# ranrandy/gaussian-splatting-mpm

Measured on AMD Instinct MI355X. Metric: MPM substeps/sec (and particles·steps/sec) + rendered fps, lego 128³ grid, higher is better.
Workload: dtype f32; 1 GPU; lego.json frame: 100 substeps + postprocess + render 800x800 SH3; particles_per_gpu=100000, particles_total=100000, n_grid=128, material=jelly, render_overlap=True, render_first=False, render_thread=True, render_async=False, parallelism=single

## Files before the change

gaussian-splatting-mpm_amd/csrc/fused.h:

```cpp

#ifndef GSMPM_FT2
#define GSMPM_FT2 7
#endif
constexpr int kFT0 = 8, kFT1 = 8, kFT2 = GSMPM_FT2;
constexpr int kFW0 = kFT0 + 4, kFW1 = kFT1 + 4, kFW2 = kFT2 + 4;
constexpr int kFWin = kFW0 * kFW1 * kFW2;
constexpr int kFTN = kFT0 * kFT1 * kFT2;

__device__ __forceinline__ int slot_loc(int w0, int w1, int w2) { return (w0 * kFW1 + w1) * kFW2 + w2; }

struct SlabWin {
  int W;
  int a[2];
  int on[2];
  float4* part[2];
  int y0[2], ny[2];
  int z0[2], nz[2];
  int* oob;
  int pass;
};

__device__ __forceinline__ int slab_window_of(const SlabWin& sw, int i) {
  if (sw.on[0] && i >= sw.a[0] && i < sw.a[0] + sw.W) return 0;
  if (sw.on[1] && i >= sw.a[1] && i < sw.a[1] + sw.W) return 1;
// ... 219 lines not shown
  int* touched;
  int* nchunk;
  int4* chunk;
  int* cbox;
  int* tbox;
  unsigned char* perm;
  int2* rcov;
  const int* tpos;
  int* rbox;
};

__device__ __forceinline__ int balanced_lane(const int* __restrict__ rcnt, int cnt, int r, int rank) {
  const int Lr = (cnt - r + 15) >> 4;
  if (rank < Lr) return rank * 16 + r;
  int o = rank - Lr;
  for (int q = 0; q < r; ++q) o += max(0, rcnt[q] - ((cnt - q + 15) >> 4));
  int acc = 0;
  for (int q = 0; q < 16; ++q) {
    const int Lq = (cnt - q + 15) >> 4, d = max(0, Lq - rcnt[q]);
    if (o < acc + d) return (rcnt[q] + (o - acc)) * 16 + q;
    acc += d;
  }
  return rank * 16 + r;
}

constexpr int kFullBox = 0 | (0 << 4) | (0 << 8) | ((kFW0 - 1) << 12) | ((kFW1 - 1) << 16) | ((kFW2 - 1) << 20);
__device__ __forceinline__ void box_unpack(int b, int (&lo)[3], int (&hi)[3]) {
#pragma unroll
  for (int d = 0; d < 3; ++d) {
    lo[d] = (b >> (4 * d)) & 15;
    hi[d] = (b >> (12 + 4 * d)) & 15;
  }
}

__device__ __forceinline__ void add_lower_tiles(const Touch& tc, const FTiles& tl, int tx, int ty, int tz, int lo) {
  const int e = threadIdx.x;
  if (e < 27) {
    const int a = e / 9 - 1, b = (e / 3) % 3 - 1, c = e % 3 - 1;
    const bool need = (a < 0 || b < 0 || c < 0) && (a >= 0 || (lo & 1)) && (b >= 0 || (lo & 2)) && (c >= 0 || (lo & 4));
    const int x = tx + a, y = ty + b, z = tz + c;
    if (need && (unsigned)x < (unsigned)tl.td0 && (unsigned)y < (unsigned)tl.td1 && (unsigned)z < (unsigned)tl.td2) {
      const int t = (x * tl.td1 + y) * tl.td2 + z;
      if (atomicCAS(&tc.tflag[t], 0, 1) == 0) {
        const int pos = atomicAdd(&tc.nchunk[1], 1);
        tc.touched[pos] = t;
        if (tc.rcov) tc.rcov[(size_t)pos * kRecStride + 27] = make_int2(1, 0);
      }
    }
  }
}

__device__ __forceinline__ void base_of(const float (&x)[3], float inv_dx, int (&b)[3]) {
#pragma unroll
  for (int d = 0; d < 3; ++d) b[d] = (int)(x[d] * inv_dx - 0.5f);
}

__device__ __forceinline__ void mark_escape_tiles(int* __restrict__ tflag, int* __restrict__ touched,
                                               int* __restrict__ ntouch, int2* __restrict__ rcov, const FTiles& tl,
                                               int ng, int b0, int b1, int b2) {
  const int lo0 = max(b0, 0), lo1 = max(b1, 0), lo2 = max(b2, 0);
  const int hi0 = min(b0 + 2, ng - 1), hi1 = min(b1 + 2, ng - 1), hi2 = min(b2 + 2, ng - 1);
  if (lo0 > hi0 || lo1 > hi1 || lo2 > hi2) return;
  for (int a = lo0 / kFT0; a <= hi0 / kFT0; ++a)
    for (int c = lo1 / kFT1; c <= hi1 / kFT1; ++c)
      for (int e = lo2 / kFT2; e <= hi2 / kFT2; ++e) {
        const int t = (a * tl.td1 + c) * tl.td2 + e;
// ... 66 lines not shown
}

__global__ __launch_bounds__(1024) void k_fold_tail(int* __restrict__ flags, float4* __restrict__ g0,
                                                    float4* __restrict__ g1, float4* __restrict__ g2, int ng) {
  __shared__ int s_f[12];
  if (threadIdx.x < 12) s_f[threadIdx.x] = flags[threadIdx.x];
  __syncthreads();
  const size_t nn = (size_t)ng * ng * ng;
  bool dirty[3] = {false, false, false};
  for (int r = 0; r < 12; ++r) dirty[r % 3] = dirty[r % 3] || s_f[r] != 0;
  float4* gb[3] = {g0, g1, g2};
  for (int b = 0; b < 3; ++b)
    if (dirty[b])
      for (size_t q = threadIdx.x; q < nn; q += 1024) gb[b][q] = make_float4(0.f, 0.f, 0.f, 0.f);
  __syncthreads();
  if (threadIdx.x < 12 && s_f[threadIdx.x]) flags[threadIdx.x] = 0;
}

__device__ __forceinline__ void load_cover27(const ChunkIn& ck, const int* __restrict__ tbox, const FTiles& tl, int ti,
                                             int tj, int tk, int* s_cov, int* s_bx) {
  const int e = threadIdx.x;
  if (e < 27) {
    const int x = ti + e / 9 - 1, y = tj + (e / 3) % 3 - 1, z = tk + e % 3 - 1;
    int c0 = 0, nc = 0, bx = 0;
    if ((unsigned)x < (unsigned)tl.td0 && (unsigned)y < (unsigned)tl.td1 && (unsigned)z < (unsigned)tl.td2) {
      const int t = (x * tl.td1 + y) * tl.td2 + z;
      const int cnt = ck.count[t];
      c0 = ck.cbase[t];
      bx = tbox[t];
      nc = (cnt + kChunk - 1) / kChunk;
    }
    s_cov[2 * e] = c0;
    s_cov[2 * e + 1] = nc;
    s_bx[e] = bx;
  }
}

struct NodeReads {
  int off[8];
  int extra;
  int live;
};
__device__ __forceinline__ void node_cover(int l0, int l1, int l2, int e, int& ci, int& loc) {
  const int sec0 = l0 < 3 ? -1 : (l0 == kFT0 - 1 ? 1 : 0);
  const int sec1 = l1 < 3 ? -1 : (l1 == kFT1 - 1 ? 1 : 0);
  const int sec2 = l2 < 3 ? -1 : (l2 == kFT2 - 1 ? 1 : 0);
  const int a = (e >> 2) ? sec0 : 0, b = ((e >> 1) & 1) ? sec1 : 0, c = (e & 1) ? sec2 : 0;
  ci = (a + 1) * 9 + (b + 1) * 3 + (c + 1);
  loc = slot_loc(l0 - a * kFT0 + 1, l1 - b * kFT1 + 1, l2 - c * kFT2 + 1);
}
__device__ __forceinline__ void node_reads(int max_chunks, const int* s_cov, const int* s_bx, int l0,
                                           int l1, int l2, NodeReads& r) {
  const int sec0 = l0 < 3 ? -1 : (l0 == kFT0 - 1 ? 1 : 0);
  const int sec1 = l1 < 3 ? -1 : (l1 == kFT1 - 1 ? 1 : 0);
  const int sec2 = l2 < 3 ? -1 : (l2 == kFT2 - 1 ? 1 : 0);
  r.extra = 0;
  r.live = 0;
  int nc[8], bx[8], c0[8], ci[8];
#pragma unroll
  for (int e = 0; e < 8; ++e) {
    const int a = (e >> 2) ? sec0 : 0, b = ((e >> 1) & 1) ? sec1 : 0, c = (e & 1) ? sec2 : 0;
    ci[e] = (a + 1) * 9 + (b + 1) * 3 + (c + 1);
    nc[e] = s_cov[2 * ci[e] + 1];
    bx[e] = s_bx[ci[e]];
    c0[e] = s_cov[2 * ci[e]];
  }
#pragma unroll
  for (int e = 0; e < 8; ++e) {
    const int ax = e >> 2, ay = (e >> 1) & 1, az = e & 1;
    const int a = ax ? sec0 : 0, b = ay ? sec1 : 0, c = az ? sec2 : 0;
    const int w0 = l0 - a * kFT0 + 1, w1 = l1 - b * kFT1 + 1, w2 = l2 - c * kFT2 + 1;
    const int q = bx[e];
    const bool on = ((!ax) | (sec0 != 0)) & ((!ay) | (sec1 != 0)) & ((!az) | (sec2 != 0)) & (nc[e] > 0) &
                    (w0 >= (q & 15)) & (w1 >= ((q >> 4) & 15)) & (w2 >= ((q >> 8) & 15)) &
                    (w0 <= ((q >> 12) & 15)) & (w1 <= ((q >> 16) & 15)) & (w2 <= ((q >> 20) & 15));
    const int loc = slot_loc(w0, w1, w2);
    r.off[e] = on ? c0[e] * kFWin + loc : max_chunks * kFWin;
    r.extra |= (on & (nc[e] > 1)) ? (1 << e) : 0;
    r.live |= on ? (1 << e) : 0;
  }
}
__device__ __forceinline__ void add4(float4& a, const float4& b) {
  a.x += b.x;
  a.y += b.y;
  a.z += b.z;
  a.w += b.w;
}
__device__ __forceinline__ void glds4(const int* src, int* lds_base) {
  __builtin_amdgcn_global_load_lds((const __attribute__((address_space(1))) void*)src,
                                   (__attribute__((address_space(3))) void*)lds_base, 4, 0, 0);
}
__device__ __forceinline__ float4 ld_slot(const float4* __restrict__ slots, int off) {
  return *(const float4*)((const char*)slots + (unsigned)off * 16u);
}
#ifndef GSMPM_STREAM_BATCH
#define GSMPM_STREAM_BATCH 8
#endif
constexpr int kStreamBatch = GSMPM_STREAM_BATCH;
__device__ __forceinline__ void node_extra(const float4* __restrict__ slots, const int* s_cov, int l0,
                                           int l1, int l2, int extra2, int zero, float4& acc) {
  int runs = extra2;
#pragma unroll
  for (int e = 0; e < 8; ++e) {
    int ci, loc;
    node_cover(l0, l1, l2, e, ci, loc);
    runs |= (((extra2 >> e) & 1) & (s_cov[2 * ci + 1] > 2)) << (8 + e);
  }
  const int sec0 = l0 < 3 ? -1 : (l0 == kFT0 - 1 ? 1 : 0);
// ... 50 lines not shown
    P = wt / kGridParts;
    part = wt - P * kGridParts;
  } else {
    const int x = b & 7, m = (b >> 3) + it * (S >> 3);
    const int u = m / kGridParts, k = u / kGridGroup;
    part = m - u * kGridParts;
    P = (k * 8 + x) * kGridGroup + (u - k * kGridGroup);
  }
}
template <bool SLAB, bool EXT = false, class GS = GridStep>
__global__ __launch_bounds__(kGridT) __attribute__((amdgpu_waves_per_eu(7, 8))) void k_grid_f(GridDims g, FTiles tl, ChunkIn ck, const int* __restrict__ tbox,
                                                    const float4* __restrict__ slots, float4* __restrict__ gacc,
                                                    float4* __restrict__ gvel, const BcTable* __restrict__ bct,
                                                    GS gs, const int* __restrict__ esc_in,
                                                    int* __restrict__ esc_clear, int* __restrict__ zc,
                                                    int* __restrict__ zf, SlabWin sw) {
  sim_prio();
  stamp(3, 0);
  const int pass = SLAB ? sw.pass : 0;
  int P0, part0;
  grid_work(blockIdx.x, 0, gridDim.x, P0, part0);
  const int i0 = min(P0, tl.ntiles - 1);
  const int* esc_p = esc_in;
  const int* cnt_p = ck.nchunk;
  const int* tch_p = ck.touched;
  asm volatile("" : "+s"(esc_p), "+s"(cnt_p), "+s"(tch_p));
  const bool pre = ck.rcov != nullptr;
  const int le = threadIdx.x;
  __shared__ int s_rec[2][64];
  __shared__ int s_box[2][64];
  __shared__ int s_tn[2];
  if (pre && threadIdx.x < 64) {
    glds4(reinterpret_cast<const int*>(ck.rcov) + (size_t)i0 * 2 * kRecStride + le, &s_rec[0][0]);
    glds4(ck.rbox + (size_t)i0 * kRecStride + (le & 31), &s_box[0][0]);
  }
  typedef const int __attribute__((address_space(1)))* gint_p;
  const int esc0 = __builtin_amdgcn_readfirstlane(*(gint_p)esc_p);
  const int cnt0 = __builtin_amdgcn_readfirstlane(((gint_p)cnt_p)[1]);
  const int T0 = __builtin_amdgcn_readfirstlane(((gint_p)tch_p)[i0]);
  const int ng = g.ng;
  const bool esc = esc0 != 0;
  const int ntouch = cnt0;
  int b = 0;
  for (int it = 0;; ++it, b ^= 1) {
    int P, part;
    grid_work(blockIdx.x, it, gridDim.x, P, part);
    if (P >= ntouch) break;
    asm volatile("s_waitcnt vmcnt(0)" ::: "memory");
    __syncthreads();
    int pn, partn;
    grid_work(blockIdx.x, it + 1, gridDim.x, pn, partn);
    if (pre && pn < ntouch && threadIdx.x < 64) {
      glds4(reinterpret_cast<const int*>(ck.rcov) + (size_t)pn * 2 * kRecStride + le, &s_rec[b ^ 1][0]);
      glds4(ck.rbox + (size_t)pn * kRecStride + (le & 31), &s_box[b ^ 1][0]);
      if (le == 0) glds4(ck.touched + pn, &s_tn[b ^ 1]);
    }
    int* s_cov = s_rec[b];
    int* s_bx = s_box[b];
    const int q = threadIdx.x + part * kGridT;
    const int l0 = q / (kFT1 * kFT2), l1 = (q / kFT2) % kFT1, l2 = q % kFT2;
    const int T = it == 0 ? T0 : pre ? s_tn[b] : ck.touched[P];
    if ((unsigned)T >= (unsigned)tl.ntiles) continue;
    int ti, tj, tk;
    ftile_decode(tl, T, ti, tj, tk);
    if (SLAB && pass != 0 && slab_tile_in_window(sw, ti) != (pass == 1)) continue;
    if (it == 0) stamp(3, 2);
    const bool tables = !pre || s_cov[54] != 0;
    if (tables) {
      load_cover27(ck, tbox, tl, ti, tj, tk, s_cov, s_bx);
      __syncthreads();
    }
    if (it == 0) stamp(3, 3);
#ifdef GSMPM_STAMPS
    if (it == 0 && threadIdx.x == 0) {
      int ncmax = 0;
      for (int e = 0; e < 27; ++e) ncmax = max(ncmax, s_cov[2 * e + 1]);
      stamp_val(3, 5, (unsigned long long)T);
      stamp_val(3, 6, (unsigned long long)(s_cov[2 * 13 + 1] | (ncmax << 16)));
      stamp_val(3, 7, (unsigned long long)part);
    }
#endif
    const int i = ti * kFT0 + l0, j = tj * kFT1 + l1, k = tk * kFT2 + l2;
    if ((unsigned)i < (unsigned)ng && (unsigned)j < (unsigned)ng && (unsigned)k < (unsigned)ng) {
      const size_t idx = ((size_t)i * ng + j) * ng + k;
      float4 a = make_float4(0.f, 0.f, 0.f, 0.f);
      NodeReads r;
      node_reads(tl.max_chunks, s_cov, s_bx, l0, l1, l2, r);
// ... 57 lines not shown
```

gaussian-splatting-mpm_amd/csrc/fused_body.inc:

```
#ifndef GSMPM_FUSED_BODY_INCLUDER
#error "fused_body.inc is the body of k_fused / k_fused_mixed: it is included inside those two kernels in fused.h only"
#endif
  constexpr bool G2P = (MODE & 1) != 0, P2G = (MODE & 2) != 0;
  constexpr bool FOLD = G2P && (MODE & 4) != 0;
  __shared__ int s_fc0[27], s_fnc[27], s_fbx[27];
  constexpr int kEscMax = kFWin / 27;
  __shared__ int s_nesc;
  __shared__ int s_eb[3][kEscMax];
  GridStep fgs{};
  bool fesc = false;
  if constexpr (FOLD) {
    fgs.dt = dt;
    fgs.dgx = dt * rare->grav[0];
    fgs.dgy = dt * rare->grav[1];
    fgs.dgz = dt * rare->grav[2];
    fgs.mask = mask_prev;
    fgs.keep = 0;
    fesc = __builtin_amdgcn_readfirstlane(*rare->esc_prev) != 0;
  }
  __shared__ unsigned long long s_acc[4 * kFWin];
  __shared__ float s_max[4];
  __shared__ int s_mxy[4], s_mz[4];
  __shared__ int s_cnt[27], s_base[27];
  __shared__ int s_rcnt[16];
  float4* s_win = reinterpret_cast<float4*>(s_acc);
  const int ng = g.ng;
  constexpr int SK = (MODE & 3) == 3 ? 0 : 1;
  sim_prio();
  stamp(SK, 0);
  const int w0 = min((int)blockIdx.x, tl.max_chunks - 1);
  const bool perm0 = use_box && tc.perm;
  const int* nch_p = ck.nchunk;
  const int4* chk_p = ck.chunk;
  const int* cbx_p = tc.cbox;
  const unsigned char* prm_p = perm0 ? tc.perm : reinterpret_cast<const unsigned char*>(tc.cbox);
  asm volatile("" : "+s"(nch_p), "+s"(chk_p), "+s"(cbx_p), "+s"(prm_p));
  typedef const int __attribute__((address_space(1)))* gint_p;
  typedef const unsigned char __attribute__((address_space(1)))* guc_p;
  const gint_p c4 = (gint_p)chk_p + 4 * (size_t)w0;
  const int r0 = c4[0], r1 = c4[1], r2 = c4[2], r3 = c4[3];
  const int bx0 = ((gint_p)cbx_p)[w0];
  const int qv0 = ((guc_p)prm_p)[perm0 ? (size_t)w0 * 256 + threadIdx.x : 0];
  const int nch = *(gint_p)nch_p;
  int4 cr_n = make_int4(r0, r1, r2, r3);
  int box_n = use_box ? bx0 : kFullBox;
  int q_n = perm0 ? qv0 : (int)threadIdx.x;
  for (int w = blockIdx.x; w < nch; w += gridDim.x) {
    const int4 cr = cr_n;
    const int cbox = box_n, q_lane = q_n;
    if (w + (int)gridDim.x < nch) {
      const int wn = w + gridDim.x;
      cr_n = ck.chunk[wn];
      box_n = use_box ? tc.cbox[wn] : kFullBox;
      q_n = (use_box && tc.perm) ? (int)tc.perm[(size_t)wn * 256 + threadIdx.x] : (int)threadIdx.x;
    }
    const int t = cr.x, first = cr.y, cnt = cr.z;
    const int k = threadIdx.x;
    const bool outside = t == tl.ntiles;
    int tx = 0, ty = 0, tz = 0;
    if (!outside) ftile_decode(tl, t, tx, ty, tz);
    const int o0 = tx * kFT0 - 1, o1 = ty * kFT1 - 1, o2 = tz * kFT2 - 1;
    int tpos_e = -1;
    const int* __restrict__ tposp = rare->tpos;
    if (tposp && !outside && k < 27) {
      const int x0 = tx - (k / 9 - 1), y0 = ty - ((k / 3) % 3 - 1), z0 = tz - (k % 3 - 1);
      if ((unsigned)x0 < (unsigned)tl.td0 && (unsigned)y0 < (unsigned)tl.td1 && (unsigned)z0 < (unsigned)tl.td2)
        tpos_e = tposp[(x0 * tl.td1 + y0) * tl.td2 + z0];
    }
    int p = -1;
    float x[3] = {0.f, 0.f, 0.f}, v[3] = {0.f, 0.f, 0.f}, C[3][3], F[3][3], m = 0.f;
    const int q = k >= cnt ? k : q_lane;
    if (k < cnt) {
      p = first + q;
#pragma unroll
      for (int d = 0; d < 3; ++d) x[d] = ps.ld(PX + d, p);
      if (G2P || MAT != 0) {
#pragma unroll
        for (int i = 0; i < 9; ++i) F[i / 3][i % 3] = ps.ld(PF + i, p);
      }
      if (P2G) m = ps.ld(PMASS, p);
      if (!G2P) {
#pragma unroll
        for (int d = 0; d < 3; ++d) v[d] = ps.ld(PV + d, p);
#pragma unroll
        for (int i = 0; i < 9; ++i) C[i / 3][i % 3] = ps.ld(PC + i, p);
      }
    }
// ... 336 lines not shown
        for (int o = 32; o > 0; o >>= 1) {
          bound = fmaxf(bound, __shfl_xor(bound, o));
          mxy |= __shfl_xor(mxy, o);
          mz |= __shfl_xor(mz, o);
        }
      }
      if ((k & 63) == 0) {
        s_max[k >> 6] = bound;
        s_mxy[k >> 6] = mxy;
        s_mz[k >> 6] = mz;
      }
      __syncthreads();
      const int res = win ? (((b[0] - o0) * kFW1 + (b[1] - o1)) * kFW2 + (b[2] - o2)) & 15 : (q & 15);
      const int rrank = (tc.perm && k < cnt) ? atomicAdd(&s_rcnt[res], 1) : 0;
      const float bmax = fmaxf(fmaxf(s_max[0], s_max[1]), fmaxf(s_max[2], s_max[3]));
      const int Mxy = s_mxy[0] | s_mxy[1] | s_mxy[2] | s_mxy[3], Mz = s_mz[0] | s_mz[1] | s_mz[2] | s_mz[3];
      const int Mx = Mxy & 0xffff, My = (unsigned)Mxy >> 16;
      const int lo_all = (Mx & 1) | ((My & 1) << 1) | ((Mz & 1) << 2);
      if (lo_all & ~cr.w) {
        Touch tr = tc;
        tr.tflag = rare->tflag;
        tr.touched = rare->touched;
        tr.nchunk = rare->nchunk;
        tr.rcov = rare->rcov;
        add_lower_tiles(tr, tl, tx, ty, tz, (lo_all | cr.w) & 7);
        if (k == 0) rare->chunk[w].w = lo_all | cr.w;
      }
      int box = kFullBox;
      if (Mx && My && Mz)
        box = (__builtin_ctz(Mx)) | (__builtin_ctz(My) << 4) | (__builtin_ctz(Mz) << 8) | ((31 - __builtin_clz(Mx)) << 12) |
              ((31 - __builtin_clz(My)) << 16) | ((31 - __builtin_clz(Mz)) << 20);
      else
        box = 0;
      if (k == 0) {
        tc.cbox[w] = box;
        rare->tbox[t] = (cr.w & 8) ? kFullBox : box;
      }
      if (tpos_e >= 0) rare->rbox[(size_t)tpos_e * kRecStride + k] = (cr.w & 8) ? kFullBox : box;
      if (cr.w & 8) box = kFullBox;
      int ebits;
      frexpf(bmax, &ebits);
      const int S = bmax > 0.f ? 50 - ebits : 0;
      if (k < cnt) {
        if (win) {
          int bb[3];
          float fx[3], ww[3][3], dw[3][3];
          bspline(x, g.inv_dx, bb, fx, ww, dw);
          p2g_scatter<MAT, kFW1, kFW2, kFWin>(s_acc + ((b[0] - o0) * kFW1 + (b[1] - o1)) * kFW2 + (b[2] - o2), fx, ww,
                                              dw, v, C, m, nvt, g, dt, ldexp(1.0, S));
        } else {
          p2g_global<MAT>(x, v, C, m, nvt, g, dt, rare->gacc);
          *rare->esc = 1;
        }
      }
      {
        const unsigned long long eb = __ballot(k < cnt && !win);
        if (eb) {
          if ((k & 63) == 0) atomicAdd(rare->esc_count, (unsigned)__popcll(eb));
          if (k < cnt && !win)
            mark_escape_tiles(rare->tflag, rare->touched, rare->nchunk + 1, rare->rcov, tl, ng, b[0], b[1], b[2]);
        }
      }
      __syncthreads();
      if (w == (int)blockIdx.x) stamp(SK, 4);
      if (tc.perm && k < cnt) tc.perm[(size_t)w * 256 + balanced_lane(s_rcnt, cnt, res, rrank)] = (unsigned char)q;
      int lo[3], hi[3];
      box_unpack(box, lo, hi);
      const int n1 = hi[1] - lo[1] + 1, n2 = hi[2] - lo[2] + 1, n12 = n1 * n2;
      const int nvol = (hi[0] - lo[0] + 1) * n12;
      const float r12 = 1.0f / (float)n12, r2 = 1.0f / (float)n2;
      const int cid = (cr.w & 16) ? (int)((unsigned)cr.w >> 5) : w;
      float4* dst = slots + (size_t)cid * kFWin;
// ... 31 lines not shown
```

gaussian-splatting-mpm_amd/csrc/mpm.hip:

```cpp
#include <hip/hip_runtime.h>
#include <dlfcn.h>


#include <algorithm>
#include <climits>
#include <cmath>
#include <cstring>
#include <map>
#include <numeric>
#include <type_traits>
#include <vector>

#include "common.h"
#include "constitutive.h"
#include <hip/hip_ext.h>

#include "mpm_common.h"
#include "svd3.h"

namespace gsmpm {

#ifndef GSMPM_REBIN_SF
#define GSMPM_REBIN_SF 20
#endif
// ... 856 lines not shown
    __syncthreads();
    if (w == (int)blockIdx.x) stamp(1, 4);
    if (p >= 0) {
      bo.ptile[p] = nt;
      bo.pslot[p] = code >= 0 ? s_base[code] + lslot : reserve(bo, nt, 1);
    }
    __syncthreads();
  }
  stamp(1, 1);
}

__global__ __launch_bounds__(256) void k_bin_all(Particles ps, GridDims g, Tiles tl, BinOut bo) {
  const int p = blockIdx.x * blockDim.x + threadIdx.x;
  if (p < ps.n) {
    float x[3];
#pragma unroll
    for (int d = 0; d < 3; ++d) x[d] = ps.ld(PX + d, p);
    int tc[3];
    const int t = tile_of(x, g, tl, tc);
    bo.ptile[p] = t;
    bo.pslot[p] = reserve(bo, t, 1);
  }
}

struct ChunkOut {
  int* cstart;
  int* cbase;
  int4* chunk;
  int* nchunk;
  const int* tflag;
  int* touched;
  int2* rcov = nullptr;
  int* tpos = nullptr;
  int td1 = 0, td2 = 0;
};

constexpr int kRecStride = 32;
__device__ __forceinline__ void write_cover_record(const ChunkOut& co, int ntiles, int E, int t, int rk,
                                                   const int* s_off, const int* s_aux, int total) {
  const int td12 = co.td1 * co.td2, td0 = ntiles / td12;
  const int tz = t % co.td2, ty = (t / co.td2) % co.td1, tx = t / td12;
  for (int e = 0; e < 27; ++e) {
    const int x = tx + e / 9 - 1, y = ty + (e / 3) % 3 - 1, z = tz + e % 3 - 1;
    int2 r = make_int2(0, 0);
    if ((unsigned)x < (unsigned)td0 && (unsigned)y < (unsigned)co.td1 && (unsigned)z < (unsigned)co.td2) {
      const int u = (x * co.td1 + y) * co.td2 + z;
      const int cnt = (u + 1 < E ? s_off[u + 1] : total) - s_off[u];
      r = make_int2(s_aux[u] & 0xffff, (cnt + kChunk - 1) / kChunk);
    }
    co.rcov[(size_t)rk * kRecStride + e] = r;
  }
  co.rcov[(size_t)rk * kRecStride + 27] = make_int2(0, 0);
}

__device__ __forceinline__ int wave_incl_scan(int v) {
  const int lane = threadIdx.x & 63;
#pragma unroll
  for (int o = 1; o < 64; o <<= 1) {
    const int y = __shfl_up(v, o);
    if (lane >= o) v += y;
  }
  return v;
}

__device__ __forceinline__ void block_scan3(const int (&v)[3], int (&o)[3], int (&tot)[3]) {
  __shared__ int s_ws[3][4];
  const int lane = threadIdx.x & 63, wave = threadIdx.x >> 6;
#pragma unroll
  for (int r = 0; r < 3; ++r) {
    const int inc = wave_incl_scan(v[r]);
    if (lane == 63) s_ws[r][wave] = inc;
    o[r] = inc - v[r];
  }
  __syncthreads();
#pragma unroll
  for (int r = 0; r < 3; ++r) {
    tot[r] = 0;
#pragma unroll
    for (int w = 0; w < 4; ++w) {
      if (w < wave) o[r] += s_ws[r][w];
      tot[r] += s_ws[r][w];
    }
  }
// ... 594 lines not shown
  int* ptile = nullptr;
  int* pslot = nullptr;
  int cur_box = 0;
  BcTable host_bc{};
  BcTable* dev_bc = nullptr;
  int n_bc = 0;
  int n_ext = 0;
  int n_mov = 0;
  float* times_dev = nullptr;
  int times_cap = 0;
  int n_rot = 0;
  RotRec host_rot[kMaxBC] = {};
  RotRec* rot_dev = nullptr;
  float* poses_dev = nullptr;
  int poses_rot = 0, poses_n = 0;
  bool has_particles = false;
  bool has_R = false;
  hipStream_t cap = nullptr;
  int resort_interval = 100;
  long since_sort = 0;
  float* planes_tmp = nullptr;
  int* orig_tmp = nullptr;
  uint32_t* sort_keys = nullptr;
  int* sort_idx = nullptr;
  unsigned* sort_tmp = nullptr;
  bool fused = true;
  FTiles ftl{};
  bool fold = false;
  bool rebin_auto = false;
  int rebin_m = 0;
  bool lane_balance = true;
  bool fuse_permute = true;
  bool cover_records = true;
  int fused_wgs = 1024;
  bool chunk_order = true;
  int ncu = 256;
  int fbpar = 0;
  int fep = 0;
  int rebin_interval = 10;
  std::map<std::vector<uint32_t>, hipGraphExec_t> graphs;
  std::map<std::vector<uint32_t>, hipGraphExec_t> graphs_alt;
  std::map<std::vector<uint32_t>, int> graph_turn;
  int graph_copies = 1;
  std::map<std::vector<uint32_t>, int> graph_box_parity;
  struct FState {
    int bpar, ep;
    float* planes;
    float* planes_alt;
    int* orig;
    int* orig_alt;
    float* cold;
    float* cold_alt;
    int* gid;
    int* gid_alt;
    long since, migrations;
  };
  std::map<std::vector<uint32_t>, FState> graph_fstate;
  bool slab = false;
  int s_lo = 0, s_hi = 0, s_margin = 2, s_interval = 10, s_rank = 0, s_world = 1;
  int s_has[2] = {0, 0};
  SlabWin sw{};
  float4* s_recv[2] = {nullptr, nullptr};
  int* d_n = nullptr;
  int* s_drift = nullptr;
  bool s_synced = false;
  bool s_rect_set = false;
// ... 92 lines not shown
static ChunkOut chunk_out(const BinLists& b) {
  return ChunkOut{b.cstart, b.cbase, b.chunk, b.nchunk, b.tflag, b.touched};
}

static ChunkIn chunk_in(gsmpm_mpm* h, int c) { return chunk_in(h->ph.b[c], h->ph.b[c].chunk); }
static ChunkOut chunk_out(gsmpm_mpm* h, int c) { return chunk_out(h->ph.b[c]); }
static BinOut bin_out(gsmpm_mpm* h, int c) {
  return BinOut{h->ph.b[c].count, h->ptile, h->pslot, h->ph.b[c].tflag, h->tl.td, h->tl.ntiles};
}

static bool use_fused(const gsmpm_mpm* h) { return h->fused; }
static const BinLists& bin_lists(const gsmpm_mpm* h, int c) { return use_fused(h) ? h->fu.b[c] : h->ph.b[c]; }

static int kernel_code(const gsmpm_mpm* h) { return h->mixed ? kMatMixed : h->mat_kernel; }
static MatIds<kMatMixed> mat_ids_of(gsmpm_mpm* h) {
  return MatIds<kMatMixed>{h->mat_ids, h->orig, (h->prm.flags & GSMPM_FLAG_JELLY_FCR) ? 4 : 0};
}

static int4* fused_records(gsmpm_mpm* h, int c) {
  return h->chunk_order ? h->fu.pchunk[c] : h->fu.b[c].chunk;
}
static ChunkIn chunk_in_f(gsmpm_mpm* h, int c) {
  ChunkIn ci = chunk_in(h->fu.b[c], fused_records(h, c));
  if (h->cover_records) {
    ci.rcov = h->fu.rcov[c];
    ci.rbox = h->fu.rbox[c];
  }
  return ci;
}
static ChunkOut chunk_out_f(gsmpm_mpm* h, int c) {
  ChunkOut co = chunk_out(h->fu.b[c]);
  co.rcov = h->fu.rcov[c];
  co.tpos = h->fu.tpos[c];
  co.td1 = h->ftl.td1;
  co.td2 = h->ftl.td2;
  return co;
}
static Touch touch_f(gsmpm_mpm* h, int c) {
  const BinLists& b = h->fu.b[c];
  return Touch{b.tflag, b.touched, b.nchunk, b.chunk, h->fu.cbox[c], h->fu.tbox[c],
               h->lane_balance ? h->fu.perm[c] : nullptr, h->fu.rcov[c],
               h->cover_records ? h->fu.tpos[c] : nullptr, h->fu.rbox[c]};
}
static BinOutF bin_out_f(gsmpm_mpm* h, int c) {
  return BinOutF{h->fu.b[c].count, h->ptile, h->pslot, h->fu.b[c].tflag, h->ftl};
}
static Tiles ftiles_flat(const gsmpm_mpm* h) { return Tiles{h->ftl.td0, h->ftl.ntiles, h->ftl.max_chunks}; }

static int p2g_grid(gsmpm_mpm* h) { return std::min(h->tl.max_chunks, 1024); }
static int g2p_grid(gsmpm_mpm* h) { return std::min(h->tl.max_chunks, 1024); }
static int grid_grid(gsmpm_mpm* h) { return std::min(h->tl.ntiles, 1024); }

template <typename F, typename... Args>
static void launch(const hipEvent_t* ev, F kernel, dim3 grid, dim3 block, hipStream_t st, Args... args) {
  if (ev)
    hipExtLaunchKernelGGL(kernel, grid, block, 0, st, ev[0], ev[1], 0, args...);
  else
    hipLaunchKernelGGL(kernel, grid, block, 0, st, args...);
}

template <int MAT>
static void launch_p2g(gsmpm_mpm* h, int c, uint32_t mask, float dt, hipStream_t st, const hipEvent_t* ev) {
  if constexpr (MAT == kMatMixed)
    launch(ev, k_p2g_mixed, dim3(p2g_grid(h)), dim3(kChunk), st, particles_of(h), h->g, h->tl, chunk_in(h, c),
           (const BcTable*)h->dev_bc, mask, dt, h->mc, h->ph.slots, h->gacc, h->nonfin_dev, mat_ids_of(h));
  else
// ... 341 lines not shown
    r.gacc_old = fold_gacc(h, ph - 2);
    r.esc_clr = fold_flag(h, ph - 3);
  }
  for (int d = 0; d < 3; ++d) r.grav[d] = (float)h->prm.gravity[d];
  r.esc_count = reinterpret_cast<unsigned*>(h->fu.esc + 3 + kFoldPhases);
  r.esc_nodes = h->fo.esc_nodes;
  r.vmax = h->slab ? nullptr : h->fu.vmax_dev;
  return r;
}
static int sync_rare(gsmpm_mpm* h, hipStream_t st) {
  bool dirty = false;
  for (int i = 0; i < 2 * kRareSlots; ++i) {
    if (i % kRareSlots >= 2 && !h->fold) continue;
    const FusedRare r = rare_of(h, i / kRareSlots, i % kRareSlots);
    if (std::memcmp(&r, &h->frare_host[i], sizeof(r)) != 0) {
      h->frare_host[i] = r;
      dirty = true;
    }
  }
  if (!dirty) return GSMPM_OK;
  GSMPM_REQUIRE(!h->capturing, "k_fused's rare arguments changed inside a capture");
  GSMPM_HIP(hipMemcpyAsync(h->fu.rare_dev, h->frare_host, sizeof(h->frare_host), hipMemcpyHostToDevice, st));
  return GSMPM_OK;
}
struct FusedLaunch {
  int c, bin, use_box, slot;
  uint32_t mask, mask_prev;
  float dt;
  float4* slots;
};
template <int MAT, int MODE>
static void launch_fused_t(gsmpm_mpm* h, const FusedLaunch& f, hipStream_t st, const hipEvent_t* ev) {
  const int xlo = h->slab ? h->s_lo - h->s_margin : INT_MIN, xhi = h->slab ? h->s_hi + h->s_margin : INT_MAX;
  if constexpr (MAT == kMatMixed)
    launch(ev, k_fused_mixed<MODE>, dim3(fused_grid(h)), dim3(256), st, particles_of(h), h->g, h->ftl,
           chunk_in_f(h, f.c), touch_f(h, f.c), f.bin, f.use_box, (const float4*)h->gvel, f.mask, f.dt, h->mc, f.slots,
           xlo, xhi, (const FusedRare*)(h->fu.rare_dev + f.c * kRareSlots + f.slot), f.mask_prev, mat_ids_of(h));
  else
    launch(ev, k_fused<MAT, MODE>, dim3(fused_grid(h)), dim3(256), st, particles_of(h), h->g, h->ftl,
           chunk_in_f(h, f.c), touch_f(h, f.c), f.bin, f.use_box, (const float4*)h->gvel, f.mask, f.dt, h->mc, f.slots,
           xlo, xhi, (const FusedRare*)(h->fu.rare_dev + f.c * kRareSlots + f.slot), f.mask_prev);
}
template <int MODE>
static void launch_fused_m(gsmpm_mpm* h, const FusedLaunch& f, hipStream_t st, const hipEvent_t* ev) {
  switch (kernel_code(h)) {
    case 0: launch_fused_t<0, MODE>(h, f, st, ev); break;
    case 1: launch_fused_t<1, MODE>(h, f, st, ev); break;
    case 2: launch_fused_t<2, MODE>(h, f, st, ev); break;
    case 3: launch_fused_t<3, MODE>(h, f, st, ev); break;
    case 5: launch_fused_t<5, MODE>(h, f, st, ev); break;
    case kMatMixed:
      if constexpr ((MODE & 4) == 0) launch_fused_t<kMatMixed, MODE>(h, f, st, ev);
      break;
    default: launch_fused_t<4, MODE>(h, f, st, ev); break;
  }
}
static int launch_fused(gsmpm_mpm* h, int mode, const FusedLaunch& f, hipStream_t st, const hipEvent_t* ev) {
  if (!h->capturing) {
    const int rc = sync_rare(h, st);
    if (rc) return rc;
  }
  switch (mode) {
    case 1: launch_fused_t<0, 1>(h, f, st, ev); break;
    case 5: launch_fused_t<0, 5>(h, f, st, ev); break;
    case 2: launch_fused_m<2>(h, f, st, ev); break;
    case 7: launch_fused_m<7>(h, f, st, ev); break;
    default: launch_fused_m<3>(h, f, st, ev); break;
  }
  GSMPM_LAUNCH_CHECK();
  return GSMPM_OK;
}
static int launch_fused(gsmpm_mpm* h, int mode, int c, bool bin, bool use_box, uint32_t mask, float dt, int ep,
                        hipStream_t st, const hipEvent_t* ev) {
// ... 485 lines not shown
  h->g.ng = prm->n_grid;
  h->g.dx = (float)(prm->grid_extent / prm->n_grid);
  h->g.inv_dx = (float)(prm->n_grid / prm->grid_extent);
  const double sin_phi = std::sin(prm->friction_angle_deg / 180.0 * 3.141592653589793);
  h->mc.alpha = (float)(std::sqrt(2.0 / 3.0) * 2.0 * sin_phi / (3.0 - sin_phi));
  h->mc.hardening = (float)prm->hardening;
  h->mc.xi = (float)prm->xi;
  h->mc.pvisc = (float)prm->plastic_viscosity;
  h->mat_kernel = prm->material;
  if (prm->material == 0 && (prm->flags & GSMPM_FLAG_JELLY_FCR)) h->mat_kernel = 4;
  h->rebin_interval = h->mat_kernel == 0 ? kRebinStressFree : kRebinStress;
  const size_t nn = (size_t)h->g.ng * h->g.ng * h->g.ng;
  auto fail = [&](hipError_t e, const char* what) {
    set_error(std::string("gsmpm_mpm_create: ") + what + ": " + hipGetErrorString(e));
    gsmpm_mpm_destroy(h);
    return GSMPM_EHIP;
  };
  hipError_t e;
#define GSMPM_TRY(call, what) \
  if ((e = (call)) != hipSuccess) return fail(e, what)
  GSMPM_TRY(alloc(h, &h->planes, (size_t)NPLANES * h->np, kMemCommon, kFillZero), "planes");
  GSMPM_TRY(alloc(h, &h->cold, (size_t)NCOLD * h->np, kMemCommon, kFillZero), "planes");
  GSMPM_TRY(alloc(h, &h->orig, (size_t)h->np, kMemCommon), "orig");
  GSMPM_TRY(alloc(h, &h->gacc, nn, kMemCommon, kFillZero), "grid acc");
  GSMPM_TRY(alloc(h, &h->gvel, nn, kMemCommon, kFillZero), "grid vel");
  h->tl.td = (h->g.ng + kTile - 1) / kTile;
  h->tl.ntiles = h->tl.td * h->tl.td * h->tl.td;
  h->tl.max_chunks = h->n / kChunk + std::min(h->tl.ntiles + 1, h->n) + 1;
  h->fused = !(prm->flags & (GSMPM_FLAG_PHASED | GSMPM_FLAG_KEEP_GRID));
  if (const char* lb = std::getenv("GSMPM_LANE_BALANCE")) h->lane_balance = lb[0] != '0';
  if (const char* gc = std::getenv("GSMPM_GRAPH_COPIES")) h->graph_copies = std::max(1, std::atoi(gc));
  if (const char* fp = std::getenv("GSMPM_FUSE_PERMUTE")) h->fuse_permute = fp[0] != '0';
  if (const char* cr = std::getenv("GSMPM_COVER_RECORDS")) h->cover_records = cr[0] != '0';
  {
    int dev = 0, ncu = 0, per_cu = 0;
    if (hipGetDevice(&dev) == hipSuccess &&
        hipDeviceGetAttribute(&ncu, hipDeviceAttributeMultiprocessorCount, dev) == hipSuccess &&
        hipOccupancyMaxActiveBlocksPerMultiprocessor(&per_cu, k_fused<0, 3>, 256, 0) == hipSuccess && ncu > 0 &&
        per_cu > 0) {
      h->ncu = ncu;
      const int resident = ncu * per_cu;
      const int rounds = (int)std::min<long long>(6, std::max<long long>(1, (long long)h->n / ((long long)resident * kChunk)));
      h->fused_wgs = resident * rounds;
      h->chunk_order = rounds == 1;
    }
    if (const char* fw = std::getenv("GSMPM_FUSED_WGS")) h->fused_wgs = std::max(1, std::atoi(fw));
    if (const char* co = std::getenv("GSMPM_CHUNK_ORDER")) h->chunk_order = co[0] != '0';
  }
  h->ftl.td0 = (h->g.ng + kFT0 - 1) / kFT0;
  h->ftl.td1 = (h->g.ng + kFT1 - 1) / kFT1;
  h->ftl.td2 = (h->g.ng + kFT2 - 1) / kFT2;
  h->ftl.ntiles = h->ftl.td0 * h->ftl.td1 * h->ftl.td2;
  h->ftl.max_chunks = h->n / kChunk + std::min(h->ftl.ntiles + 1, h->n) + 1;
  if (h->fused && sizeof(float4) * (size_t)(h->ftl.max_chunks + 1) * kFWin > 0xffffffffull) h->fused = false;
  if (const char* fo = std::getenv("GSMPM_FOLD")) h->fold = h->fused && fo[0] != '0';
  if (const char* ra = std::getenv("GSMPM_REBIN_AUTO")) h->rebin_auto = h->fused && ra[0] != '0';
  if (!h->fused) {
    GSMPM_TRY(alloc(h, &h->ph.slots, (size_t)(h->tl.max_chunks + 1) * kWin, kMemPhased, kFillZero,
                    (size_t)h->tl.max_chunks * kWin),
              "chunk slots");
    for (BinLists& b : h->ph.b)
      GSMPM_TRY(alloc_bin_lists(h, b, h->tl.ntiles, h->tl.max_chunks, kMemPhased), "bin lists");
  } else {
    FusedBufs& f = h->fu;
    const size_t nt = (size_t)h->ftl.ntiles, mc = (size_t)h->ftl.max_chunks;
    GSMPM_TRY(alloc(h, &f.slots, (mc + 1) * kFWin, kMemFused, kFillZero, mc * kFWin), "fused slots");
    for (int c = 0; c < 2; ++c) {
      GSMPM_TRY(alloc_bin_lists(h, f.b[c], h->ftl.ntiles, h->ftl.max_chunks, kMemFused), "bin lists");
      GSMPM_TRY(alloc(h, &f.cbox[c], mc, kMemFused), "boxes");
      GSMPM_TRY(alloc(h, &f.pchunk[c], mc, kMemFused, kFillZero), "ordered chunks");
      GSMPM_TRY(alloc(h, &f.tbox[c], nt, kMemFused), "boxes");
      GSMPM_TRY(alloc(h, &f.rcov[c], kRecStride * nt, kMemFused, kFillZero), "cover records");
      GSMPM_TRY(alloc(h, &f.rbox[c], kRecStride * nt, kMemFused, kFillZero), "cover boxes");
      GSMPM_TRY(alloc(h, &f.tpos[c], nt, kMemFused, kFillOnes), "touched positions");
      GSMPM_TRY(alloc(h, &f.perm[c], mc * 256, kMemFused, kFillZero), "lane balance");
    }
    GSMPM_TRY(alloc(h, &f.planes_alt, (size_t)NPLANES * h->np, kMemFused, kFillZero), "planes");
    GSMPM_TRY(alloc(h, &f.orig_alt, (size_t)h->np, kMemFused), "orig");
    GSMPM_TRY(alloc(h, &f.esc, 4 + kFoldPhases, kMemFused, kFillZero), "escape flags");
    GSMPM_TRY(alloc(h, &f.vmax_dev, 1, kMemFused, kFillZero), "vmax");
    GSMPM_TRY(alloc_host(h, &f.vmax_host, 1), "pinned vmax");
    *f.vmax_host = 0.f;
    GSMPM_TRY(alloc(h, &f.rare_dev, 2 * kRareSlots, kMemFused, kFillZero), "rare args");
    if (h->fold) {
      GSMPM_TRY(alloc(h, &h->fo.slots2, (mc + 1) * kFWin, kMemFold, kFillZero, mc * kFWin), "fused slots");
      for (float4*& g : h->fo.gacc) GSMPM_TRY(alloc(h, &g, nn, kMemFold, kFillZero), "grid acc");
      GSMPM_TRY(alloc(h, &h->fo.esc_nodes, 27 * (size_t)h->np, kMemFold), "escape nodes");
      for (int*& t : h->fo.tbox2) GSMPM_TRY(alloc(h, &t, nt, kMemFold, kFillZero), "boxes");
    }
  }
  const int scan_tiles = std::max(h->tl.ntiles, h->ftl.ntiles) + 1;
  GSMPM_TRY(alloc(h, &h->scan_part, (size_t)div_up(scan_tiles, 1024), kMemCommon), "scan partials");
  GSMPM_TRY(alloc(h, &h->ptile, (size_t)h->np, kMemCommon), "ptile");
  GSMPM_TRY(alloc(h, &h->pslot, (size_t)h->np, kMemCommon), "pslot");
  GSMPM_TRY(alloc(h, &h->dev_bc, 1, kMemCommon), "bc table");
  GSMPM_TRY(hipStreamCreateWithFlags(&h->cap, hipStreamNonBlocking), "hipStreamCreate");
  GSMPM_TRY(alloc_host(h, &h->nonfin_host, 16, hipHostMallocMapped), "pinned non-finite word");
  *(volatile int*)h->nonfin_host = 0;
  GSMPM_TRY(hipHostGetDevicePointer((void**)&h->nonfin_dev, h->nonfin_host, 0), "hipHostGetDevicePointer");
  h->host_bc = BcTable{};
  GSMPM_TRY(hipMemcpy(h->dev_bc, &h->host_bc, sizeof(BcTable), hipMemcpyHostToDevice), "hipMemcpy bc");
  GSMPM_TRY(hipDeviceSynchronize(), "init");
#undef GSMPM_TRY
  *out = h;
  return GSMPM_OK;
}
// ... 840 lines not shown
```

Baseline: 3.528 billion particle-substeps/s.

## Use per-axis bitmask boxes and hull-merged multi-chunk boxes to skip empty node reads

Cover boxes are now stored as per-axis occupancy bitmasks (x|y<<16, z), so the node-read test becomes shifts and ANDs instead of six range comparisons. Tiles covered by several chunks no longer fall back to a full box. Each chunk ORs its mask into the record atomically, and the running box becomes the hull of the chunk boxes, so more empty window nodes are skipped when gathering. This doubles the cover-box record stride, adds atomics and zeroing writes, and loads 64 ints per record instead of 32. It is enabled by default except in fold mode.

Measured after the change: 3.684 billion particle-substeps/s, median of 6. 4.4% higher.

```diff
diff --git a/gaussian-splatting-mpm_amd/csrc/fused.h b/gaussian-splatting-mpm_amd/csrc/fused.h
--- a/gaussian-splatting-mpm_amd/csrc/fused.h
+++ b/gaussian-splatting-mpm_amd/csrc/fused.h
@@ -275,6 +275,21 @@
     hi[d] = (b >> (12 + 4 * d)) & 15;
   }
 }
+__device__ __forceinline__ int box_hull(int a, int b) {
+  int r = 0;
+#pragma unroll
+  for (int d = 0; d < 3; ++d) {
+    r |= min((a >> (4 * d)) & 15, (b >> (4 * d)) & 15) << (4 * d);
+    r |= max((a >> (12 + 4 * d)) & 15, (b >> (12 + 4 * d)) & 15) << (12 + 4 * d);
+  }
+  return r;
+}
+__device__ __forceinline__ int2 box_masks(int b) {
+  int lo[3], hi[3];
+  box_unpack(b, lo, hi);
+  const int mx = (2 << hi[0]) - (1 << lo[0]), my = (2 << hi[1]) - (1 << lo[1]), mz = (2 << hi[2]) - (1 << lo[2]);
+  return make_int2(mx | (my << 16), mz);
+}
 
 __device__ __forceinline__ void add_lower_tiles(const Touch& tc, const FTiles& tl, int tx, int ty, int tz, int lo) {
   const int e = threadIdx.x;
@@ -407,7 +422,9 @@
     }
     s_cov[2 * e] = c0;
     s_cov[2 * e + 1] = nc;
-    s_bx[e] = bx;
+    const int2 bm = box_masks(bx);
+    s_bx[e] = bm.x;
+    s_bx[32 + e] = bm.y;
   }
 }
 
@@ -431,13 +448,14 @@
   const int sec2 = l2 < 3 ? -1 : (l2 == kFT2 - 1 ? 1 : 0);
   r.extra = 0;
   r.live = 0;
-  int nc[8], bx[8], c0[8], ci[8];
+  int nc[8], bxy[8], bz[8], c0[8], ci[8];
 #pragma unroll
   for (int e = 0; e < 8; ++e) {
     const int a = (e >> 2) ? sec0 : 0, b = ((e >> 1) & 1) ? sec1 : 0, c = (e & 1) ? sec2 : 0;
     ci[e] = (a + 1) * 9 + (b + 1) * 3 + (c + 1);
     nc[e] = s_cov[2 * ci[e] + 1];
-    bx[e] = s_bx[ci[e]];
+    bxy[e] = s_bx[ci[e]];
+    bz[e] = s_bx[32 + ci[e]];
     c0[e] = s_cov[2 * ci[e]];
   }
 #pragma unroll
@@ -445,10 +463,8 @@
     const int ax = e >> 2, ay = (e >> 1) & 1, az = e & 1;
     const int a = ax ? sec0 : 0, b = ay ? sec1 : 0, c = az ? sec2 : 0;
     const int w0 = l0 - a * kFT0 + 1, w1 = l1 - b * kFT1 + 1, w2 = l2 - c * kFT2 + 1;
-    const int q = bx[e];
-    const bool on = ((!ax) | (sec0 != 0)) & ((!ay) | (sec1 != 0)) & ((!az) | (sec2 != 0)) & (nc[e] > 0) &
-                    (w0 >= (q & 15)) & (w1 >= ((q >> 4) & 15)) & (w2 >= ((q >> 8) & 15)) &
-                    (w0 <= ((q >> 12) & 15)) & (w1 <= ((q >> 16) & 15)) & (w2 <= ((q >> 20) & 15));
+    const int inb = ((unsigned)bxy[e] >> w0) & ((unsigned)bxy[e] >> (16 + w1)) & ((unsigned)bz[e] >> w2) & 1;
+    const bool on = ((!ax) | (sec0 != 0)) & ((!ay) | (sec1 != 0)) & ((!az) | (sec2 != 0)) & (nc[e] > 0) & (inb != 0);
     const int loc = slot_loc(w0, w1, w2);
     r.off[e] = on ? c0[e] * kFWin + loc : max_chunks * kFWin;
     r.extra |= (on & (nc[e] > 1)) ? (1 << e) : 0;
@@ -565,7 +581,7 @@
   __shared__ int s_tn[2];
   if (pre && threadIdx.x < 64) {
     glds4(reinterpret_cast<const int*>(ck.rcov) + (size_t)i0 * 2 * kRecStride + le, &s_rec[0][0]);
-    glds4(ck.rbox + (size_t)i0 * kRecStride + (le & 31), &s_box[0][0]);
+    glds4(ck.rbox + (size_t)i0 * kBoxStride + le, &s_box[0][0]);
   }
   typedef const int __attribute__((address_space(1)))* gint_p;
   const int esc0 = __builtin_amdgcn_readfirstlane(*(gint_p)esc_p);
@@ -585,7 +601,7 @@
     grid_work(blockIdx.x, it + 1, gridDim.x, pn, partn);
     if (pre && pn < ntouch && threadIdx.x < 64) {
       glds4(reinterpret_cast<const int*>(ck.rcov) + (size_t)pn * 2 * kRecStride + le, &s_rec[b ^ 1][0]);
-      glds4(ck.rbox + (size_t)pn * kRecStride + (le & 31), &s_box[b ^ 1][0]);
+      glds4(ck.rbox + (size_t)pn * kBoxStride + le, &s_box[b ^ 1][0]);
       if (le == 0) glds4(ck.touched + pn, &s_tn[b ^ 1]);
     }
     int* s_cov = s_rec[b];
diff --git a/gaussian-splatting-mpm_amd/csrc/fused_body.inc b/gaussian-splatting-mpm_amd/csrc/fused_body.inc
--- a/gaussian-splatting-mpm_amd/csrc/fused_body.inc
+++ b/gaussian-splatting-mpm_amd/csrc/fused_body.inc
@@ -28,8 +28,9 @@
   constexpr int SK = (MODE & 3) == 3 ? 0 : 1;
   sim_prio();
   stamp(SK, 0);
+  const bool boxed = (use_box & 1) != 0, dense_box = (use_box & 2) != 0;
   const int w0 = min((int)blockIdx.x, tl.max_chunks - 1);
-  const bool perm0 = use_box && tc.perm;
+  const bool perm0 = boxed && tc.perm;
   const int* nch_p = ck.nchunk;
   const int4* chk_p = ck.chunk;
   const int* cbx_p = tc.cbox;
@@ -43,7 +44,7 @@
   const int qv0 = ((guc_p)prm_p)[perm0 ? (size_t)w0 * 256 + threadIdx.x : 0];
   const int nch = *(gint_p)nch_p;
   int4 cr_n = make_int4(r0, r1, r2, r3);
-  int box_n = use_box ? bx0 : kFullBox;
+  int box_n = boxed ? bx0 : kFullBox;
   int q_n = perm0 ? qv0 : (int)threadIdx.x;
   for (int w = blockIdx.x; w < nch; w += gridDim.x) {
     const int4 cr = cr_n;
@@ -51,8 +52,8 @@
     if (w + (int)gridDim.x < nch) {
       const int wn = w + gridDim.x;
       cr_n = ck.chunk[wn];
-      box_n = use_box ? tc.cbox[wn] : kFullBox;
-      q_n = (use_box && tc.perm) ? (int)tc.perm[(size_t)wn * 256 + threadIdx.x] : (int)threadIdx.x;
+      box_n = boxed ? tc.cbox[wn] : kFullBox;
+      q_n = (boxed && tc.perm) ? (int)tc.perm[(size_t)wn * 256 + threadIdx.x] : (int)threadIdx.x;
     }
     const int t = cr.x, first = cr.y, cnt = cr.z;
     const int k = threadIdx.x;
@@ -455,12 +456,23 @@
               ((31 - __builtin_clz(My)) << 16) | ((31 - __builtin_clz(Mz)) << 20);
       else
         box = 0;
+      const bool multi = (cr.w & 8) != 0;
       if (k == 0) {
         tc.cbox[w] = box;
-        rare->tbox[t] = (cr.w & 8) ? kFullBox : box;
-      }
-      if (tpos_e >= 0) rare->rbox[(size_t)tpos_e * kRecStride + k] = (cr.w & 8) ? kFullBox : box;
-      if (cr.w & 8) box = kFullBox;
+        rare->tbox[t] = multi ? kFullBox : box;
+      }
+      if (tpos_e >= 0) {
+        int* rb = rare->rbox + (size_t)tpos_e * kBoxStride + k;
+        const int2 bm = box_masks(multi && !dense_box ? kFullBox : box);
+        if (multi && dense_box) {
+          atomicOr(rb, bm.x);
+          atomicOr(rb + 32, bm.y);
+        } else {
+          rb[0] = bm.x;
+          rb[32] = bm.y;
+        }
+      }
+      if (multi) box = dense_box ? box_hull(cbox, box) : kFullBox;
       int ebits;
       frexpf(bmax, &ebits);
       const int S = bmax > 0.f ? 50 - ebits : 0;
diff --git a/gaussian-splatting-mpm_amd/csrc/mpm.hip b/gaussian-splatting-mpm_amd/csrc/mpm.hip
--- a/gaussian-splatting-mpm_amd/csrc/mpm.hip
+++ b/gaussian-splatting-mpm_amd/csrc/mpm.hip
@@ -912,10 +912,12 @@
   int* touched;
   int2* rcov = nullptr;
   int* tpos = nullptr;
+  int* rbox = nullptr;
   int td1 = 0, td2 = 0;
 };
 
 constexpr int kRecStride = 32;
+constexpr int kBoxStride = 64;
 __device__ __forceinline__ void write_cover_record(const ChunkOut& co, int ntiles, int E, int t, int rk,
                                                    const int* s_off, const int* s_aux, int total) {
   const int td12 = co.td1 * co.td2, td0 = ntiles / td12;
@@ -929,6 +931,8 @@
       r = make_int2(s_aux[u] & 0xffff, (cnt + kChunk - 1) / kChunk);
     }
     co.rcov[(size_t)rk * kRecStride + e] = r;
+    co.rbox[(size_t)rk * kBoxStride + e] = 0;
+    co.rbox[(size_t)rk * kBoxStride + 32 + e] = 0;
   }
   co.rcov[(size_t)rk * kRecStride + 27] = make_int2(0, 0);
 }
@@ -1589,6 +1593,7 @@
   bool lane_balance = true;
   bool fuse_permute = true;
   bool cover_records = true;
+  bool dense_box = true;
   int fused_wgs = 1024;
   bool chunk_order = true;
   int ncu = 256;
@@ -1747,6 +1752,7 @@
   ChunkOut co = chunk_out(h->fu.b[c]);
   co.rcov = h->fu.rcov[c];
   co.tpos = h->fu.tpos[c];
+  co.rbox = h->fu.rbox[c];
   co.td1 = h->ftl.td1;
   co.td2 = h->ftl.td2;
   return co;
@@ -2154,13 +2160,14 @@
 template <int MAT, int MODE>
 static void launch_fused_t(gsmpm_mpm* h, const FusedLaunch& f, hipStream_t st, const hipEvent_t* ev) {
   const int xlo = h->slab ? h->s_lo - h->s_margin : INT_MIN, xhi = h->slab ? h->s_hi + h->s_margin : INT_MAX;
+  const int use_box = f.use_box | (h->dense_box && !h->fold ? 2 : 0);
   if constexpr (MAT == kMatMixed)
     launch(ev, k_fused_mixed<MODE>, dim3(fused_grid(h)), dim3(256), st, particles_of(h), h->g, h->ftl,
-           chunk_in_f(h, f.c), touch_f(h, f.c), f.bin, f.use_box, (const float4*)h->gvel, f.mask, f.dt, h->mc, f.slots,
+           chunk_in_f(h, f.c), touch_f(h, f.c), f.bin, use_box, (const float4*)h->gvel, f.mask, f.dt, h->mc, f.slots,
            xlo, xhi, (const FusedRare*)(h->fu.rare_dev + f.c * kRareSlots + f.slot), f.mask_prev, mat_ids_of(h));
   else
     launch(ev, k_fused<MAT, MODE>, dim3(fused_grid(h)), dim3(256), st, particles_of(h), h->g, h->ftl,
-           chunk_in_f(h, f.c), touch_f(h, f.c), f.bin, f.use_box, (const float4*)h->gvel, f.mask, f.dt, h->mc, f.slots,
+           chunk_in_f(h, f.c), touch_f(h, f.c), f.bin, use_box, (const float4*)h->gvel, f.mask, f.dt, h->mc, f.slots,
            xlo, xhi, (const FusedRare*)(h->fu.rare_dev + f.c * kRareSlots + f.slot), f.mask_prev);
 }
 template <int MODE>
@@ -2712,6 +2719,7 @@
   if (const char* gc = std::getenv("GSMPM_GRAPH_COPIES")) h->graph_copies = std::max(1, std::atoi(gc));
   if (const char* fp = std::getenv("GSMPM_FUSE_PERMUTE")) h->fuse_permute = fp[0] != '0';
   if (const char* cr = std::getenv("GSMPM_COVER_RECORDS")) h->cover_records = cr[0] != '0';
+  if (const char* db = std::getenv("GSMPM_DENSE_BOX")) h->dense_box = db[0] != '0';
   {
     int dev = 0, ncu = 0, per_cu = 0;
     if (hipGetDevice(&dev) == hipSuccess &&
@@ -2751,7 +2759,7 @@
       GSMPM_TRY(alloc(h, &f.pchunk[c], mc, kMemFused, kFillZero), "ordered chunks");
       GSMPM_TRY(alloc(h, &f.tbox[c], nt, kMemFused), "boxes");
       GSMPM_TRY(alloc(h, &f.rcov[c], kRecStride * nt, kMemFused, kFillZero), "cover records");
-      GSMPM_TRY(alloc(h, &f.rbox[c], kRecStride * nt, kMemFused, kFillZero), "cover boxes");
+      GSMPM_TRY(alloc(h, &f.rbox[c], kBoxStride * nt, kMemFused, kFillZero), "cover boxes");
       GSMPM_TRY(alloc(h, &f.tpos[c], nt, kMemFused, kFillOnes), "touched positions");
       GSMPM_TRY(alloc(h, &f.perm[c], mc * 256, kMemFused, kFillZero), "lane balance");
     }
```
